# konstantineder/montecarlo-risk-engine

Measured on AMD Instinct MI355X. Metric: path-steps/sec at 1M paths x 250 steps; PV/CVA rel-error vs CPU ref, higher is better.
Workload: dtype f64

## Files before the change

montecarlo-risk-engine_amd/csrc/k1_paths.hip:

```cpp
#include "mcx_device.h"

namespace {


#ifndef MCX_K1_PPL
#define MCX_K1_PPL 1
#endif
template <int NSLOT, int NZ, bool INJECT, int SIG>
__global__ __launch_bounds__(MCX_BLOCK) void k1_paths(const K1Args a)
{
    constexpr int PPL = INJECT ? 1 : MCX_K1_PPL;
    __shared__ double bm_lds[INJECT ? 2 : MCX_BM_LDS_DOUBLES];
    const double* tab = nullptr;
    if (!INJECT) { mcx_bm_load(bm_lds); tab = bm_lds; }
    const int64_t tid = (int64_t)blockIdx.x * MCX_BLOCK + threadIdx.x;
    const int64_t half = (int64_t)gridDim.x * MCX_BLOCK;
    if (tid >= a.n) return;
    double reg[PPL][2 * NSLOT];
    int64_t idx[PPL];
    bool live[PPL];
#pragma unroll
    for (int q = 0; q < PPL; ++q) {
        idx[q] = tid + q * half;
        live[q] = idx[q] < a.n;
        if (!live[q]) idx[q] = a.n - 1;
        sim_init_state<NSLOT, SIG>(a, reg[q], idx[q]);
    }
    for (int t = 0; t < a.n_initial_store; ++t)
#pragma unroll
        for (int q = 0; q < PPL; ++q) if (live[q]) sim_store_state<NSLOT, SIG>(a, t, idx[q], reg[q]);
    const mcx_bm_coef bc = mcx_bm_coef_load();
    const mcx_bm_vconst vc = mcx_bm_vconst_make(bc);
    for (int k = 0; k < a.n_steps; ++k) {
        int st;
        if constexpr (INJECT || SIG == SIG_GENERIC) {
#pragma unroll
            for (int q = 0; q < PPL; ++q)
                sim_substep<NSLOT, NZ, INJECT, SIG>(a, k, a.path_offset + (uint64_t)idx[q], idx[q], reg[q], tab, a.seed, bc, &vc);
            st = ldk(&a.steps[k].store_idx);
        } else {
            const StepData<NSLOT, NZ> sdat = sim_step_load<NSLOT, NZ, SIG>(a, k);
            __builtin_amdgcn_sched_barrier(0);
            uint64_t path[PPL];
            uint32_t st_q[PPL];
            double zz[PPL][NZ], uu[PPL];
#pragma unroll
            for (int q = 0; q < PPL; ++q) { path[q] = a.path_offset + (uint64_t)idx[q]; st_q[q] = (uint32_t)k; }
            const bool rare = sim_draw_n<PPL, NZ, SIG, 7>(a, st_q, path, zz, uu, tab, a.seed, bc, vc);
            if (__builtin_expect(__any(rare), 0)) {
#pragma unroll
                for (int q = 0; q < PPL; ++q) sim_draw<NZ, false, SIG, 7, true>(a, k, path[q], idx[q], zz[q], uu[q], tab, a.seed, bc, &vc);
            }
            st = -1;
#pragma unroll
            for (int q = 0; q < PPL; ++q) st = sim_apply_loaded<NSLOT, NZ, SIG>(a, sdat, reg[q], zz[q], uu[q]);
        }
        if (st >= 0)
#pragma unroll
            for (int q = 0; q < PPL; ++q) if (live[q]) sim_store_state<NSLOT, SIG>(a, st, idx[q], reg[q], a.aux + (int64_t)k * NSLOT * MCX_AUX);
    }
}

template <int NSLOT, int NZ, int SIG>
int launch_k1(const K1Args& a, bool inject, hipStream_t s)
{
    const int ppl = inject ? 1 : MCX_K1_PPL;
    const int grid = (int)((a.n + (int64_t)MCX_BLOCK * ppl - 1) / ((int64_t)MCX_BLOCK * ppl));
    if (inject) hipLaunchKernelGGL((k1_paths<NSLOT, NZ, true, SIG>), dim3(grid), dim3(MCX_BLOCK), 0, s, a);
    else hipLaunchKernelGGL((k1_paths<NSLOT, NZ, false, SIG>), dim3(grid), dim3(MCX_BLOCK), 0, s, a);
    return 0;
}

__global__ __launch_bounds__(MCX_BLOCK) void k1_rng_draws(uint64_t seed, uint64_t path0, int64_t n, uint32_t step, uint32_t draw,
                                                          uint32_t* __restrict__ words, double* __restrict__ u, double* __restrict__ z)
{
    __shared__ double bm_lds[MCX_BM_LDS_DOUBLES];
    mcx_bm_load(bm_lds);
    const mcx_bm_coef bc = mcx_bm_coef_load();
    for (int64_t i = (int64_t)blockIdx.x * MCX_BLOCK + threadIdx.x; i < n; i += (int64_t)gridDim.x * MCX_BLOCK) {
        const uint64_t path = path0 + (uint64_t)i;
        if (words) {
            uint32_t w0, w1, w2, w3;
            philox4x32_10((uint32_t)path, (uint32_t)(path >> 32), step, draw, (uint32_t)seed, (uint32_t)(seed >> 32), w0, w1, w2, w3);
            words[i] = w0; words[n + i] = w1; words[2 * n + i] = w2; words[3 * n + i] = w3;
            if (u) { u[i] = u53(w0, w1); u[n + i] = u53(w2, w3); }
        }
        if (z) {
            double ua, z0, z1;
            draw_pair<true>(seed, path, step, draw, ua, z0, z1, bm_lds, bc);
            z[i] = z0; z[n + i] = z1;
        }
    }
}

template <int BMB>
__global__ __launch_bounds__(MCX_BLOCK) void k1_box_muller(const uint32_t* __restrict__ words, int64_t n, double* __restrict__ u,
                                                          double* __restrict__ z)
{
    __shared__ double bm_lds[MCX_BM_LDS_DOUBLES_B(BMB)];
    mcx_bm_load<BMB>(bm_lds);
    const mcx_bm_coef bc = mcx_bm_coef_load();
    const mcx_bm_vconst vc = mcx_bm_vconst_make<BMB>(bc);
    for (int64_t i = (int64_t)blockIdx.x * MCX_BLOCK + threadIdx.x; i < n; i += (int64_t)gridDim.x * MCX_BLOCK) {
        const uint32_t w0 = words[i], w1 = words[n + i], w2 = words[2 * n + i], w3 = words[3 * n + i];
        double ua, z0, z1;
        pair_from_words<true, BMB>(w0, w1, w2, w3, ua, z0, z1, bm_lds, bc, &vc);
        if (u) { u[i] = ua; u[n + i] = u53(w2, w3); }
        z[i] = z0; z[n + i] = z1;
    }
}

}

extern "C" int mcx_box_muller(mcx_handle* h, const uint32_t* d_words, int64_t n, int32_t table_bits, double* d_u, double* d_z, void* stream)
{
    if (!h || !d_words || !d_z) return -1;
    if (table_bits != 7 && table_bits != 10) MCX_FAIL(h, -2, "mcx_box_muller: table_bits must be 7 or 10");
    if (n <= 0) return 0;
    const int grid = mcx_grid_for(n, MCX_BLOCK, 2048);
    if (table_bits == 7) hipLaunchKernelGGL(k1_box_muller<7>, dim3(grid), dim3(MCX_BLOCK), 0, (hipStream_t)stream, d_words, n, d_u, d_z);
    else hipLaunchKernelGGL(k1_box_muller<10>, dim3(grid), dim3(MCX_BLOCK), 0, (hipStream_t)stream, d_words, n, d_u, d_z);
    MCX_HIP(h, hipGetLastError());
    return 0;
}

extern "C" int mcx_rng_draws(mcx_handle* h, uint64_t seed, uint64_t path0, int64_t n, uint32_t step, uint32_t draw,
                             uint32_t* d_words, double* d_u, double* d_z, void* stream)
{
    if (!h) return -1;
    if (n <= 0) return 0;
    if (d_u && !d_words) MCX_FAIL(h, -2, "mcx_rng_draws: d_u needs d_words");
// ... 149 lines not shown
```

montecarlo-risk-engine_amd/csrc/kf_lean.hip:

```cpp
#include <cstdlib>
#include <map>
#include <utility>

#include "kf_common.h"

namespace {

template <int NSLOT, int PPL>
__device__ __forceinline__ void lean_date_cva(const FastDateCvaLds* __restrict__ rp, const double (&reg)[PPL][2 * NSLOT], double (&cva)[PPL],
                                              const double* __restrict__ etab)
{
    const mcx_expq_coef ec = mcx_expq_load(mcx_region_zero());
    const FastDateCvaLds r = *rp;
    double xe[2 * PPL], ev[2 * PPL];
#pragma unroll
    for (int q = 0; q < PPL; ++q) {
        xe[2 * q] = fma(r.m_s1, reg[q][FDC_S_REG], fma(r.m_n1, reg[q][FDC_NI_REG], r.m_c0));
        xe[2 * q + 1] = fma(r.c_c1, reg[q][FDC_C_REG], r.c_c0);
    }
    mcx_exp_tab_n<2 * PPL>(xe, ev, etab, ec);
#pragma unroll
    for (int q = 0; q < PPL; ++q) {
        const double x = fma(r.x_d, reg[q][FDC_X_REG], r.x_a);
        double p = 0.0;
        p += fma(fma(r.row0[2], x, r.row0[1]), x, r.row0[0]);
        p += fma(fma(r.row1[2], x, r.row1[1]), x, r.row1[0]);
        const double w = r.m_b * ev[2 * q];
        const double cs = fma(r.c_b, ev[2 * q + 1], r.c_a);
        cva[q] = fma(fmax(p, 0.0), w * (1.0 - cs), cva[q]);
    }
}

#define MCX_LEAN_WAVES 4
template <int NSLOT, int NZ, bool INJECT, int SIG, int PPL, bool SIMULATE, int DK = 0>
__global__ __launch_bounds__(MCX_BLOCK, MCX_LEAN_WAVES) void kf_lean(const FusedArgs)
{
    static_assert(DK == 0 || (SIG == SIG_VAS_CIR_E && SIMULATE && !INJECT), "the cva-date kernel simulates the Vasicek + CIR++ signature");
    constexpr int NREG = 2 * NSLOT;
    constexpr int TILE = MCX_BLOCK * PPL;
    extern __shared__ double lds[];
    KArgs& a0 = kargs_region(0);
    const int n_rec = a0.n_rec;
    const int64_t n = a0.k1.n;
    for (int q = threadIdx.x; q < 9 * n_rec; q += MCX_BLOCK) lds[q] = 0.0;
    FastDateCvaLds* const dlds = (FastDateCvaLds*)(lds + ((9 * n_rec + 1) & ~1));
    if constexpr (DK == 1) {
        const FastDateCva* __restrict__ dc = a0.cva_dates;
        const double* __restrict__ cf = a0.coeffs;
        const int n_dates = a0.n_dates;
        for (int q = threadIdx.x; q < 16 * n_dates; q += MCX_BLOCK) {
            const int t = q >> 4, e = q & 15;
            double v;
            if (e < FDC_HEAD) {
                v = ((const double*)(dc + t))[e];
            } else {
                const int off = e < FDC_HEAD + 3 ? dc[t].coeff_off0 : dc[t].coeff_off1;
                v = off >= 0 ? cf[off + (e - FDC_HEAD) % 3] : 0.0;
            }
            ((double*)dlds)[q] = v;
        }
    }
    constexpr int BMB = SIG == SIG_VAS_CIR_E ? 10 : 7;
    constexpr int BM = (INJECT || !SIMULATE) ? 0 : MCX_BM_LDS_DOUBLES_B(BMB);
    __shared__ double tab_lds[BM + MCX_EXP_LDS_DOUBLES];
    const double* tab = nullptr;
    const double* etab = tab_lds + BM;
    mcx_exp_tab_load(tab_lds + BM);
    if (BM) { mcx_bm_load<BMB>(tab_lds); tab = tab_lds; }
    __syncthreads();
    const int64_t tiles = (n + TILE - 1) / TILE;
    double n_block = 0.0;

    for (int64_t tile = blockIdx.x; tile < tiles; tile += gridDim.x) {
        const bool first_tile = tile == (int64_t)blockIdx.x;
        int64_t i[PPL];
        bool live[PPL];
        uint64_t path[PPL];
        double reg[PPL][NREG];
        double cfs[PPL], cva[PPL];
        int est[PPL];
        int n_init, n_steps;
        {
            KArgs& a = kargs_region(mcx_region_zero());
            const auto& k = a.k1;
#pragma unroll
            for (int q = 0; q < PPL; ++q) {
                const int64_t i_raw = tile * TILE + q * MCX_BLOCK + threadIdx.x;
                live[q] = i_raw < n;
                i[q] = live[q] ? i_raw : n - 1;
                path[q] = k.path_offset + (uint64_t)i[q];
                sim_init_state<NSLOT, SIG>(k, reg[q]);
                cfs[q] = 0.0; cva[q] = 0.0;
                est[q] = a.init_state[0];
            }
            const int64_t rest = n - tile * TILE;
            n_block += (double)(rest < TILE ? rest : TILE);
            n_init = k.n_initial_store; n_steps = k.n_steps;
        }
        if (SIMULATE) {
        int step = 0, t_init = 0;
#pragma unroll 1
        while (true) {
            const bool init = t_init < n_init;
            if (!init && step >= n_steps) break;
            int st = init ? t_init : -1;
            t_init += init ? 1 : 0;
            {
                const int zr0 = mcx_region_zero();
                const auto& k = kargs_region(zr0).k1;
                const uint64_t seed = k.seed;
                const mcx_bm_coef bc = mcx_bm_coef_load(zr0);
                const mcx_bm_vconst vc = mcx_bm_vconst_make<BMB>(bc);
#pragma unroll 1
                while (st < 0 && step < n_steps) {
                    if constexpr (SIG == SIG_GENERIC) {
#pragma unroll
                        for (int q = 0; q < PPL; ++q) sim_substep<NSLOT, NZ, INJECT, SIG, BMB, true>(k, step, path[q], i[q], reg[q], tab, seed, bc, &vc);
                        st = ldk(&k.steps[step].store_idx);
                    } else {
                        double zz[PPL][NZ], uu[PPL];
                        bool rare = false;
                        const StepData<NSLOT, NZ> sdat = sim_step_load<NSLOT, NZ, SIG>(k, step);
                        __builtin_amdgcn_sched_barrier(0);
                        if constexpr (INJECT) {
#pragma unroll
                            for (int q = 0; q < PPL; ++q) sim_draw<NZ, true, SIG, BMB>(k, step, path[q], i[q], zz[q], uu[q], tab, seed, bc, &vc);
                        } else {
                            uint32_t st_q[PPL];
#pragma unroll
                            for (int q = 0; q < PPL; ++q) st_q[q] = (uint32_t)step;
                            rare = sim_draw_n<PPL, NZ, SIG, BMB>(k, st_q, path, zz, uu, tab, seed, bc, vc);
                        }
                        if (!INJECT && __builtin_expect(__any(rare), 0)) {
#pragma unroll
                            for (int q = 0; q < PPL; ++q) sim_draw<NZ, false, SIG, BMB, true>(k, step, path[q], i[q], zz[q], uu[q], tab, seed, bc, &vc);
                        }
#pragma unroll
                        for (int q = 0; q < PPL; ++q) st = sim_apply_loaded<NSLOT, NZ, SIG, true>(k, sdat, reg[q], zz[q], uu[q]);
                    }
                    ++step;
                }
            }
            if (st >= 0) {
                if constexpr (DK == 1) lean_date_cva<NSLOT, PPL>(dlds + st, reg, cva, etab);
                else lean_date<NSLOT, SIG, PPL, true>(st, i, live, first_tile, lds, reg, cfs, cva, est, etab);
            }
        }
        } else {
            auto load_row = [&](int t, double (&dst)[PPL][NREG]) {
                const auto& k = kargs_region(0).k1;
                const int D = k.n_state;
#pragma unroll
                for (int q = 0; q < PPL; ++q)
#pragma unroll
                    for (int sl = 0; sl < NSLOT; ++sl) {
                        const bool bs = sig_kind(SIG, sl) >= 0 ? sig_is_bs(SIG, sl) : (k.slots[sl].kind == MCX_MODEL_BS);
                        const int c = k.slots[sl].state_off;
                        dst[q][2 * sl] = k.paths[((int64_t)t * D + c) * k.ld + i[q]];
                        dst[q][2 * sl + 1] = bs ? 0.0 : k.paths[((int64_t)t * D + c + 1) * k.ld + i[q]];
                    }
            };
            const int n_dates = kargs_region(0).n_dates;
            double bufb[PPL][NREG];
            load_row(0, reg);
            load_row(n_dates > 1 ? 1 : 0, bufb);
#pragma unroll 1
            for (int t = 0; t < n_dates; t += 2) {
                lean_date<NSLOT, SIG, PPL, false>(t, i, live, first_tile, lds, reg, cfs, cva, est, etab);
                if (t + 2 < n_dates) load_row(t + 2, reg);
                if (t + 1 < n_dates) {
                    lean_date<NSLOT, SIG, PPL, false>(t + 1, i, live, first_tile, lds, bufb, cfs, cva, est, etab);
                    if (t + 3 < n_dates) load_row(t + 3, bufb);
                }
            }
        }
        {
            KArgs& a = kargs_region(mcx_region_zero());
#pragma unroll
            for (int q = 0; q < PPL; ++q) if (a.cfs && live[q]) a.cfs[i[q]] = cfs[q];
            if (a.rec_pv[0] >= 0) lean_record<PPL>(cfs, live, a.rec_pv[0], n_rec, first_tile, lds);
            if (a.rec_cva[0] >= 0) {
                const double lgd = a.lgd[0];
                double cc[PPL];
#pragma unroll
                for (int q = 0; q < PPL; ++q) cc[q] = cva[q] * lgd;
                lean_record<PPL>(cc, live, a.rec_cva[0], n_rec, first_tile, lds);
            }
        }
    }
    __syncthreads();
    for (int r = threadIdx.x; r < n_rec; r += MCX_BLOCK) {
        double s1 = 0.0, s2 = 0.0;
        for (int w = 0; w < 4; ++w) { s1 += lds[n_rec + (w * n_rec + r) * 2]; s2 += lds[n_rec + (w * n_rec + r) * 2 + 1]; }
        double* dst = a0.partials + ((int64_t)blockIdx.x * n_rec + r) * 4;
        dst[0] = n_block; dst[1] = lds[r]; dst[2] = s1; dst[3] = s2;
    }
}

template <int NSLOT, int NZ, int SIG, int PPL>
int launch_lean_shape(const FusedArgs& a, int n_cu, bool inject, bool simulate, hipStream_t s)
{
    const int64_t tiles = (a.k1.n + MCX_BLOCK * PPL - 1) / (MCX_BLOCK * PPL);
    const size_t lds = sizeof(double) * (size_t)((9 * a.n_rec + 1) & ~1);
    const size_t lds_cva = lds + sizeof(FastDateCvaLds) * (size_t)a.n_dates;
    auto residency = [&](auto kernel, size_t bytes) {
        thread_local std::map<std::pair<const void*, size_t>, int> cache;
        const auto key = std::make_pair((const void*)kernel, bytes);
        auto it = cache.find(key);
        if (it == cache.end()) {
            int per_cu = 0;
            if (hipOccupancyMaxActiveBlocksPerMultiprocessor(&per_cu, kernel, MCX_BLOCK, bytes) != hipSuccess || per_cu < 1) per_cu = 1;
            it = cache.emplace(key, per_cu < MCX_LEAN_WAVES ? per_cu : MCX_LEAN_WAVES).first;
        }
        return (int64_t)it->second * n_cu;
    };
    auto sized = [&](int64_t resident) {
        if (tiles <= resident) return (int)tiles;
        const int64_t per = (tiles + resident - 1) / resident;
        return (int)((tiles + per - 1) / per);
    };
    int grid;
    if (!simulate) {
        auto kern = kf_lean<NSLOT, NZ, false, SIG, PPL, false>;
        grid = sized(residency(kern, lds));
// ... 73 lines not shown
```

montecarlo-risk-engine_amd/csrc/mcx_device.h:

```cpp
#pragma once
#include "mcx_internal.h"

struct K1Args {
    mcx_slot slots[MCX_MAX_SLOTS];
    double init_state[MCX_MAX_STATE];
    const mcx_step* __restrict__ steps;
    const double* __restrict__ chol;
    const double* __restrict__ aux;
    double* __restrict__ paths;
    const double* __restrict__ inject_z;
    const double* __restrict__ inject_u;
    const double* __restrict__ init_paths;
    int64_t n, ld;
    uint64_t seed, path_offset;
    int32_t scheme, n_steps, n_state, n_initial_store, flags, n_uniform;
};

static inline void mcx_fill_k1_args(const mcx_sim* sim, uint64_t seed, uint64_t path_offset, int64_t n_paths, int64_t ld,
                                    double* d_paths, const double* d_inject_z, const double* d_inject_u, K1Args* a)
{
    const mcx_sim_desc& d = sim->desc;
    memset(a, 0, sizeof(*a));
    for (int s = 0; s < d.n_slots; ++s) a->slots[s] = d.slots[s];
    for (int c = 0; c < d.n_state; ++c) a->init_state[c] = d.init_state[c];
    a->steps = sim->d_steps; a->chol = sim->d_chol; a->aux = sim->d_aux;
    a->paths = d_paths; a->inject_z = d_inject_z; a->inject_u = d_inject_u;
    a->n = n_paths; a->ld = ld; a->seed = seed; a->path_offset = path_offset;
    a->scheme = d.scheme; a->n_steps = d.n_steps; a->n_state = d.n_state; a->n_initial_store = d.n_initial_store;
    a->flags = d.flags; a->n_uniform = d.n_uniform;
}

__device__ __forceinline__ void philox4x32_10(uint32_t c0, uint32_t c1, uint32_t c2, uint32_t c3, uint32_t k0, uint32_t k1,
                                              uint32_t& o0, uint32_t& o1, uint32_t& o2, uint32_t& o3)
{
#pragma unroll
    for (int r = 0; r < 10; ++r) {
        const uint64_t p0 = (uint64_t)0xD2511F53u * c0;
        const uint64_t p1 = (uint64_t)0xCD9E8D57u * c2;
        const uint32_t n0 = __builtin_amdgcn_bitop3_b32((uint32_t)(p1 >> 32), c1, k0, 0x96);
        const uint32_t n2 = __builtin_amdgcn_bitop3_b32((uint32_t)(p0 >> 32), c3, k1, 0x96);
        c1 = (uint32_t)p1;
        c3 = (uint32_t)p0;
        c0 = n0;
        c2 = n2;
        k0 += 0x9E3779B9u;
        k1 += 0xBB67AE85u;
    }
    o0 = c0; o1 = c1; o2 = c2; o3 = c3;
}

__device__ __forceinline__ double u53(uint32_t lo, uint32_t hi, const mcx_bm_vconst* vc = nullptr)
{
    if (vc) return fma((double)hi, vc->s32, fma((double)(lo >> 11), vc->s53, vc->c54));
    return fma((double)hi, 0x1.0p-32, fma((double)(lo >> 11), 0x1.0p-53, 0x1.0p-54));
}

struct DevBridge {
    uint64_t seed, path_offset;
    const double* const* inject;
    int64_t ld;
};

__device__ __forceinline__ double dev_barrier_event(const DevEvent& e, const DevTerm* __restrict__ terms, const double* __restrict__ coeffs,
                                                    const DevBridge* __restrict__ bridge, const double* __restrict__ paths, int64_t D,
                                                    int64_t ld, int64_t i, double num)
{
    const int types = (int)e.aux[3];
    const int t1 = types & 7, t2 = types >> 3;
    const bool with_bridge = e.aux[0] == 5.0;
    double mx = -1.0e300, mn = 1.0e300, keep1 = 1.0, keep2 = 1.0, prev1 = 0.0, prev2 = 0.0;
    double c = 0.0;
    int draw_id = 0;
    DevBridge br = {0, 0, nullptr, 0};
    const double* __restrict__ inj = nullptr;
    if (with_bridge) {
        c = ldk(coeffs + e.coeff_off);
        draw_id = (int)ldk(coeffs + e.coeff_off + 1);
        br = ldk_struct(bridge);
        if (br.inject) inj = br.inject[draw_id];
    }
    AtomCache bc = {-1, -1, 0.0};
    for (int j = e.term_begin; j < e.term_end; ++j) {
        const double s = dev_atom_cached(ldk_struct(&terms[j]).atom, paths, D, ld, i, bc);
        mx = fmax(mx, s); mn = fmin(mn, s);
        if (with_bridge) {
            const double cur1 = mcx_log(s / e.aux[1]), cur2 = t2 ? mcx_log(s / e.aux[2]) : 0.0;
            if (j > e.term_begin) {
                const int k = j - e.term_begin - 1;
                for (int bi = 0; bi < (t2 ? 2 : 1); ++bi) {
                    const double p = mcx_exp(c * (bi ? prev2 * cur2 : prev1 * cur1));
                    double u;
                    if (inj) u = inj[(int64_t)(2 * k + bi) * br.ld + i];
                    else {
                        uint32_t w0, w1, w2, w3;
                        const uint64_t path = br.path_offset + (uint64_t)i;
                        philox4x32_10((uint32_t)path, (uint32_t)(path >> 32), (uint32_t)k, 0x80000000u | (uint32_t)(2 * draw_id + bi),
                                      (uint32_t)br.seed, (uint32_t)(br.seed >> 32), w0, w1, w2, w3);
                        u = u53(w0, w1);
                    }
                    const double hit = fmin(fmax((p - u + 0.05) / 0.1, 0.0), 1.0);
                    if (bi) keep2 *= 1.0 - hit; else keep1 *= 1.0 - hit;
                }
            }
            prev1 = cur1; prev2 = cur2;
        }
    }
    double pay = fmax(e.sign * (dev_atom(e.x, paths, D, ld, i) - e.strike), 0.0) * dev_barrier_ind(t1, e.aux[1], mx, mn);
    if (with_bridge) pay *= (t1 <= 2) ? keep1 : 1.0 - keep1;
    if (t2) {
        pay *= dev_barrier_ind(t2, e.aux[2], mx, mn);
        if (with_bridge) pay *= (t2 <= 2) ? keep2 : 1.0 - keep2;
    }
    return pay / num;
}

template <bool TAB = false, int BMB = 7, bool GUARD = true>
__device__ __forceinline__ bool pair_from_words(uint32_t w0, uint32_t w1, uint32_t w2, uint32_t w3, double& ua, double& z0, double& z1,
                                                const double* __restrict__ tab, const mcx_bm_coef& bc, const mcx_bm_vconst* vc = nullptr)
{
    ua = u53(w0, w1, vc);
    double s, c, r;
    if (TAB) {
        const double r2 = mcx_m2log_tab<BMB>(ua, tab, bc, vc);
        if (!GUARD) r = mcx_sqrt_gp(r2);
        else if (__builtin_expect(__any(w1 == 0xffffffffu), 0)) r = ua < 1.0 ? mcx_sqrt_g(r2) : 0.0;
        else r = mcx_sqrt_gp(r2);
        const int j = (int)(w3 >> (32 - BMB));
        const double ur = u53(w2, w3 & ((1u << (32 - BMB)) - 1u), vc);
        mcx_sincos2pi_tab<BMB>(ur, j, tab, s, c, bc, vc);
    } else {
        r = mcx_sqrt(-2.0 * mcx_log(ua));
        mcx_sincos2pi(u53(w2, w3), s, c);
    }
    z0 = r * c;
    z1 = r * s;
    return w1 == 0xffffffffu;
}

template <bool TAB = false, int BMB = 7, bool GUARD = true>
__device__ __forceinline__ bool draw_pair(uint64_t seed, uint64_t path, uint32_t step, uint32_t draw, double& ua, double& z0, double& z1,
                                          const double* __restrict__ tab, const mcx_bm_coef& bc, const mcx_bm_vconst* vc = nullptr)
{
    uint32_t w0, w1, w2, w3;
    philox4x32_10((uint32_t)path, (uint32_t)(path >> 32), step, draw, (uint32_t)seed, (uint32_t)(seed >> 32), w0, w1, w2, w3);
    return pair_from_words<TAB, BMB, GUARD>(w0, w1, w2, w3, ua, z0, z1, tab, bc, vc);
}

template <bool TAB = false>
__device__ __forceinline__ void draw_pair(uint64_t seed, uint64_t path, uint32_t step, uint32_t draw, double& ua, double& z0, double& z1,
                                          const double* __restrict__ tab = nullptr)
{
    const mcx_bm_coef bc = mcx_bm_coef_load();
    draw_pair<TAB>(seed, path, step, draw, ua, z0, z1, tab, bc);
}

__device__ __forceinline__ double degree_of_truth(double x, bool fuzzy, double eps)
{
    if (!fuzzy) return x > 0.0 ? 1.0 : 0.0;
    const double v = (x + eps) / (2.0 * eps);
    return fmin(fmax(v, 0.0), 1.0);
}

struct AuxPtr {
    const double* __restrict__ p;
    __device__ __forceinline__ double operator[](int i) const { return ldk(p + i); }
    __device__ __forceinline__ mcx_aux_drv drv() const { return ldk_struct((const mcx_aux_drv*)(p + MCX_AUX_C0)); }
};
struct AuxRegs {
    double v[MCX_AUX];
    __device__ __forceinline__ double operator[](int i) const { return v[i]; }
    __device__ __forceinline__ mcx_aux_drv drv() const { mcx_aux_drv d; d.c0 = v[MCX_AUX_C0]; d.c1 = v[MCX_AUX_C1]; d.c2 = v[MCX_AUX_C2]; return d; }
};

template <int KIND, int SCHEME, bool POS = false, class SL, class AUX>
__device__ __forceinline__ void step_slot(const SL& sl, int scheme_rt, int flags, double dt, double sq,
                                          const AUX& aux, double& s0, double& s1, double zc0, double zc1, double u)
{
    const auto* p = sl.p;
    const int scheme = SCHEME >= 0 ? SCHEME : scheme_rt;
    switch (KIND >= 0 ? KIND : sl.kind) {
    case MCX_MODEL_BS:
        if (scheme == MCX_SCHEME_ANALYTICAL) {
            s0 = s0 * mcx_exp(aux[0] + (zc0 - aux[1]));
        } else {
            const mcx_aux_drv dc = aux.drv();
            s0 = fma(s0, fma(dc.c2, zc0, dc.c0), s0);
        }
        break;
    case MCX_MODEL_VASICEK: {
        const double r = s0;
        s1 = s1 + r * dt;
        if (scheme == MCX_SCHEME_ANALYTICAL) s0 = (p[2] + (r - p[2]) * aux[0]) + zc0;
        else {
            const mcx_aux_drv dc = aux.drv();
            s0 = fma(dc.c1, r, s0);
            s0 = fma(dc.c2, zc0, s0);
            s0 = s0 + dc.c0;
        }
        break;
    }
    case MCX_MODEL_HW: {
        const double r = s0;
        s1 = s1 + r * dt;
        if (scheme == MCX_SCHEME_ANALYTICAL) s0 = r * aux[0] + aux[1] + zc0;
        else s0 = r + (aux[0] - p[3] * r) * dt + p[1] * sq * zc0;
        break;
    }
    case MCX_MODEL_CIRPP: {
        const double y = s0;
        const double sy = POS ? mcx_sqrt_gp(y) : mcx_sqrt_g(y);
        const mcx_aux_drv dc = aux.drv();
// ... 68 lines not shown
    default: break;
    }
}


enum { SIG_GENERIC = 0, SIG_VAS_CIR_E = 1, SIG_BS_A = 2, SIG_BS_E = 3, SIG_HESTON_QE = 4, SIG_HESTON_E = 5,
       SIG_VAS_E = 6, SIG_VAS_A = 7, SIG_BS_VAS_CIRDET_E = 8 };

__host__ __device__ constexpr int sig_kind(int sig, int slot)
{
    return sig == SIG_VAS_CIR_E ? (slot == 0 ? MCX_MODEL_VASICEK : MCX_MODEL_CIRPP)
         : (sig == SIG_BS_A || sig == SIG_BS_E) ? MCX_MODEL_BS
         : (sig == SIG_HESTON_QE || sig == SIG_HESTON_E) ? MCX_MODEL_HESTON
         : (sig == SIG_VAS_E || sig == SIG_VAS_A) ? MCX_MODEL_VASICEK
         : sig == SIG_BS_VAS_CIRDET_E ? (slot == 0 ? MCX_MODEL_BS : slot == 1 ? MCX_MODEL_VASICEK : MCX_MODEL_CIRPP_DET)
         : -1;
}
__host__ __device__ constexpr int sig_scheme(int sig)
{
    return (sig == SIG_VAS_CIR_E || sig == SIG_BS_E || sig == SIG_HESTON_E || sig == SIG_VAS_E || sig == SIG_BS_VAS_CIRDET_E) ? MCX_SCHEME_EULER
         : (sig == SIG_BS_A || sig == SIG_VAS_A) ? MCX_SCHEME_ANALYTICAL
         : sig == SIG_HESTON_QE ? MCX_SCHEME_QE : -1;
}
__host__ __device__ constexpr bool sig_is_bs(int sig, int slot) { return sig_kind(sig, slot) == MCX_MODEL_BS; }

static inline int mcx_sim_signature(const mcx_sim_desc& d)
{
    auto k = [&](int s) { return d.slots[s].kind; };
    if (d.n_slots == 2 && k(0) == MCX_MODEL_VASICEK && k(1) == MCX_MODEL_CIRPP && d.scheme == MCX_SCHEME_EULER) return SIG_VAS_CIR_E;
    if (d.n_slots == 3 && k(0) == MCX_MODEL_BS && k(1) == MCX_MODEL_VASICEK && k(2) == MCX_MODEL_CIRPP_DET && d.scheme == MCX_SCHEME_EULER)
        return SIG_BS_VAS_CIRDET_E;
    if (d.n_slots == 1) {
        if (k(0) == MCX_MODEL_BS) return d.scheme == MCX_SCHEME_ANALYTICAL ? SIG_BS_A : d.scheme == MCX_SCHEME_EULER ? SIG_BS_E : SIG_GENERIC;
        if (k(0) == MCX_MODEL_HESTON) return d.scheme == MCX_SCHEME_QE ? SIG_HESTON_QE : d.scheme == MCX_SCHEME_EULER ? SIG_HESTON_E : SIG_GENERIC;
        if (k(0) == MCX_MODEL_VASICEK) return d.scheme == MCX_SCHEME_EULER ? SIG_VAS_E : d.scheme == MCX_SCHEME_ANALYTICAL ? SIG_VAS_A : SIG_GENERIC;
    }
    return SIG_GENERIC;
}

__device__ __forceinline__ AuxPtr aux_of_slot(const double* __restrict__ ax, int s) { return AuxPtr{ax + s * MCX_AUX}; }
template <int NSLOT>
__device__ __forceinline__ const AuxRegs& aux_of_slot(const AuxRegs (&ax)[NSLOT], int s) { return ax[s]; }

template <int NSLOT, int NZ, int SIG, int S, bool POS = false, class KA, class AX>
__device__ __forceinline__ void step_slots(const KA& k, const mcx_step& sp, const AX& ax,
                                           double (&reg)[2 * NSLOT], const double (&zc)[NZ], double u)
{
    if constexpr (S < NSLOT) {
        const double zc0 = (NSLOT == 1) ? zc[0] : zc[S < NZ ? S : 0];
        const double zc1 = (NSLOT == 1 && NZ > 1) ? zc[NZ > 1 ? 1 : 0] : 0.0;
        step_slot<sig_kind(SIG, S), sig_scheme(SIG), POS>(k.slots[S], k.scheme, k.flags | k.slots[S].flags, sp.dt, sp.sqrt_dt,
                                                      aux_of_slot(ax, S), reg[2 * S], reg[2 * S + 1], zc0, zc1, u);
        step_slots<NSLOT, NZ, SIG, S + 1, POS>(k, sp, ax, reg, zc, u);
    }
}

template <int NZ, bool INJECT, int SIG, int BMB = 7, bool GUARD = true, class KA>
__device__ __forceinline__ bool sim_draw(const KA& k, int step, uint64_t path, int64_t i, double (&z)[NZ], double& u,
                                         const double* __restrict__ tab, uint64_t seed, const mcx_bm_coef& bc, const mcx_bm_vconst* vc = nullptr)
{
    u = 0.0;
    bool rare = false;
    if (INJECT) {
#pragma unroll
        for (int j = 0; j < NZ; ++j) z[j] = k.inject_z[((int64_t)step * NZ + j) * k.ld + i];
        if (k.n_uniform) u = k.inject_u[(int64_t)step * k.ld + i];
    } else {
        double ua;
#pragma unroll
        for (int q = 0; q < (NZ + 1) / 2; ++q) {
            double z0, z1;
            rare |= draw_pair<true, BMB, GUARD>(seed, path, (uint32_t)step, (uint32_t)q, ua, z0, z1, tab, bc, vc);
            z[2 * q] = z0;
            if (2 * q + 1 < NZ) z[2 * q + 1] = z1;
        }
        if (sig_scheme(SIG) == MCX_SCHEME_QE || (sig_scheme(SIG) < 0 && k.n_uniform)) {
            double z0, z1;
            draw_pair<false>(seed, path, (uint32_t)step, (uint32_t)((NZ + 1) / 2), u, z0, z1, nullptr, bc);
        }
    }
    return rare;
}

template <int PPL>
__device__ __forceinline__ void philox4x32_10_n(const uint64_t (&path)[PPL], const uint32_t (&step)[PPL], uint32_t draw, uint64_t seed,
                                                uint32_t (&o0)[PPL], uint32_t (&o1)[PPL], uint32_t (&o2)[PPL], uint32_t (&o3)[PPL])
{
    uint32_t c0[PPL], c1[PPL], c2[PPL], c3[PPL];
#pragma unroll
    for (int q = 0; q < PPL; ++q) { c0[q] = (uint32_t)path[q]; c1[q] = (uint32_t)(path[q] >> 32); c2[q] = step[q]; c3[q] = draw; }
    uint32_t k0 = (uint32_t)seed, k1 = (uint32_t)(seed >> 32);
#pragma unroll
    for (int r = 0; r < 10; ++r) {
#pragma unroll
        for (int q = 0; q < PPL; ++q) {
            const uint64_t p0 = (uint64_t)0xD2511F53u * c0[q];
            const uint64_t p1 = (uint64_t)0xCD9E8D57u * c2[q];
            const uint32_t n0 = __builtin_amdgcn_bitop3_b32((uint32_t)(p1 >> 32), c1[q], k0, 0x96);
            const uint32_t n2 = __builtin_amdgcn_bitop3_b32((uint32_t)(p0 >> 32), c3[q], k1, 0x96);
            c1[q] = (uint32_t)p1; c3[q] = (uint32_t)p0; c0[q] = n0; c2[q] = n2;
        }
        k0 += 0x9E3779B9u;
        k1 += 0xBB67AE85u;
    }
#pragma unroll
    for (int q = 0; q < PPL; ++q) { o0[q] = c0[q]; o1[q] = c1[q]; o2[q] = c2[q]; o3[q] = c3[q]; }
}

template <int PPL, int BMB>
__device__ __forceinline__ bool draw_pairs_staged(uint64_t seed, const uint64_t (&path)[PPL], const uint32_t (&step)[PPL], uint32_t draw,
                                                  double (&z0)[PPL], double (&z1)[PPL], const double* __restrict__ tab,
                                                  const mcx_bm_coef& C, const mcx_bm_vconst& vc)
{
    constexpr int N = 1 << BMB, LOG_TERMS = mcx_bm_shape<BMB>::LOG_TERMS;
    uint32_t w0[PPL], w1[PPL], w2[PPL], w3[PPL];
    philox4x32_10_n<PPL>(path, step, draw, seed, w0, w1, w2, w3);
    double m[PPL], ed[PPL], ps[PPL], pc[PPL];
    int e[PPL];
    mcx_d2 tc[PPL], sc[PPL];
#pragma unroll
    for (int q = 0; q < PPL; ++q) {
        const double ua = u53(w0[q], w1[q], &vc);
        m[q] = __builtin_amdgcn_frexp_mant(ua);
        e[q] = __builtin_amdgcn_frexp_exp(ua);
        const int jl = (__double2hiint(m[q]) >> (20 - BMB)) & (N - 1);
        tc[q] = ((const mcx_d2*)tab)[jl];
        sc[q] = ((const mcx_d2*)(tab + 2 * N))[(int)(w3[q] >> (32 - BMB))];
    }
    __builtin_amdgcn_sched_barrier(0);
#pragma unroll
    for (int q = 0; q < PPL; ++q) {
        const double ur = u53(w2[q], w3[q] & ((1u << (32 - BMB)) - 1u), &vc);
        const double d = fma(ur, 6.28318530717958647692, vc.trig_off);
        const double d2 = d * d;
        double qs, qc;
        if constexpr (mcx_bm_shape<BMB>::TRIG_TERMS == 3) {
            qs = fma(fma(vc.sin_head, d2, C.c[7]), d2, C.c[6]);
            qc = fma(fma(vc.cos_head, d2, C.c[10]), d2, C.c[9]);
        } else {
            qs = fma(vc.sin_head, d2, C.c[6]);
            qc = fma(vc.cos_head, d2, C.c[9]);
        }
        ps[q] = fma(d * d2, qs, d);
        pc[q] = fma(d2, qc, 1.0);
        ed[q] = (double)e[q];
    }
    __builtin_amdgcn_sched_barrier(0);
    bool rare = false;
#pragma unroll
    for (int q = 0; q < PPL; ++q) {
        const double s = fma(m[q], tc[q].x, 2.0);
        double p = vc.log_head;
#pragma unroll
        for (int k = LOG_TERMS - 2; k >= 0; --k) p = fma(p, s, C.c[k]);
        const double r2 = fma(ed[q], -2.0 * 6.93147180559945309417e-01, tc[q].y) + fma(s * s, p, s);
        const double r = mcx_sqrt_gp(r2);
        const double sn = fma(sc[q].x, pc[q], sc[q].y * ps[q]);
        const double cs = fma(-sc[q].x, ps[q], sc[q].y * pc[q]);
        z0[q] = r * cs;
        z1[q] = r * sn;
        rare |= w1[q] == 0xffffffffu;
    }
    return rare;
}

template <int PPL, int NZ, int SIG, int BMB, class KA>
__device__ __forceinline__ bool sim_draw_n(const KA& k, const uint32_t (&step)[PPL], const uint64_t (&path)[PPL], double (&z)[PPL][NZ], double (&u)[PPL],
                                           const double* __restrict__ tab, uint64_t seed, const mcx_bm_coef& bc, const mcx_bm_vconst& vc)
{
    bool rare = false;
#pragma unroll
    for (int dq = 0; dq < (NZ + 1) / 2; ++dq) {
        double a[PPL], b[PPL];
        rare |= draw_pairs_staged<PPL, BMB>(seed, path, step, (uint32_t)dq, a, b, tab, bc, vc);
#pragma unroll
        for (int q = 0; q < PPL; ++q) { z[q][2 * dq] = a[q]; if (2 * dq + 1 < NZ) z[q][2 * dq + 1] = b[q]; }
    }
#pragma unroll
    for (int q = 0; q < PPL; ++q) {
        u[q] = 0.0;
        if (sig_scheme(SIG) == MCX_SCHEME_QE || (sig_scheme(SIG) < 0 && k.n_uniform)) {
            double t0, t1;
            draw_pair<false>(seed, path[q], step[q], (uint32_t)((NZ + 1) / 2), u[q], t0, t1, nullptr, bc);
        }
    }
    return rare;
}

template <int NSLOT, int NZ, int SIG, bool POS = false, class KA>
__device__ __forceinline__ int sim_apply(const KA& k, int step, double (&reg)[2 * NSLOT], const double (&z)[NZ], double u)
{
    const mcx_step sp = ldk_struct(&k.steps[step]);
    double zc[NZ];
    constexpr bool UNIT_L00 = sig_scheme(SIG) == MCX_SCHEME_EULER || sig_scheme(SIG) == MCX_SCHEME_QE;
    const double* __restrict__ L = UNIT_L00 ? k.chol : k.chol + (int64_t)sp.chol_idx * NZ * NZ;
#pragma unroll
    for (int r = 0; r < NZ; ++r) {
        double acc = (UNIT_L00 && r == 0) ? z[0] : ldk(L + r * NZ) * z[0];
#pragma unroll
        for (int c = 1; c <= r; ++c) acc = fma(ldk(L + r * NZ + c), z[c], acc);
        zc[r] = acc;
    }
    const double* __restrict__ ax = k.aux + (int64_t)step * NSLOT * MCX_AUX;
    step_slots<NSLOT, NZ, SIG, 0, POS>(k, sp, ax, reg, zc, u);
    return sp.store_idx;
}

template <int NSLOT, int NZ>
struct StepData {
    mcx_step sp;
    double L[NZ * NZ];
    AuxRegs ax[NSLOT];
};
template <int NSLOT, int NZ, int SIG, class KA>
__device__ __forceinline__ StepData<NSLOT, NZ> sim_step_load(const KA& k, int step)
{
    StepData<NSLOT, NZ> d;
    d.sp = ldk_struct(&k.steps[step]);
    constexpr bool UNIT_L00 = sig_scheme(SIG) == MCX_SCHEME_EULER || sig_scheme(SIG) == MCX_SCHEME_QE;
    const double* __restrict__ L = UNIT_L00 ? k.chol : k.chol + (int64_t)d.sp.chol_idx * NZ * NZ;
#pragma unroll
    for (int q = 0; q < NZ * NZ; ++q) d.L[q] = ldk(L + q);
    struct P2 { double v[2]; };
    struct P4 { double v[4]; };
    static_assert(MCX_AUX == 8, "aux row layout");
    const double* __restrict__ ax = k.aux + (int64_t)step * NSLOT * MCX_AUX;
#pragma unroll
    for (int s = 0; s < NSLOT; ++s) {
        const P2 a = ldk_struct((const P2*)(ax + s * MCX_AUX)), b = ldk_struct((const P2*)(ax + s * MCX_AUX + 2));
        const P4 c = ldk_struct((const P4*)(ax + s * MCX_AUX + 4));
        d.ax[s].v[0] = a.v[0]; d.ax[s].v[1] = a.v[1]; d.ax[s].v[2] = b.v[0]; d.ax[s].v[3] = b.v[1];
#pragma unroll
        for (int q = 0; q < 4; ++q) d.ax[s].v[4 + q] = c.v[q];
    }
    return d;
}
template <int NSLOT, int NZ, int SIG, bool POS = false, class KA>
__device__ __forceinline__ int sim_apply_loaded(const KA& k, const StepData<NSLOT, NZ>& d, double (&reg)[2 * NSLOT], const double (&z)[NZ], double u)
{
    double zc[NZ];
    constexpr bool UNIT_L00 = sig_scheme(SIG) == MCX_SCHEME_EULER || sig_scheme(SIG) == MCX_SCHEME_QE;
#pragma unroll
    for (int r = 0; r < NZ; ++r) {
        double acc = (UNIT_L00 && r == 0) ? z[0] : d.L[r * NZ] * z[0];
#pragma unroll
        for (int c = 1; c <= r; ++c) acc = fma(d.L[r * NZ + c], z[c], acc);
        zc[r] = acc;
    }
    step_slots<NSLOT, NZ, SIG, 0, POS>(k, d.sp, d.ax, reg, zc, u);
    return d.sp.store_idx;
}

template <int NSLOT, int NZ, bool INJECT, int SIG, int BMB = 7, bool POS = false, class KA>
__device__ __forceinline__ void sim_substep(const KA& k, int step, uint64_t path, int64_t i, double (&reg)[2 * NSLOT],
                                            const double* __restrict__ tab, uint64_t seed, const mcx_bm_coef& bc, const mcx_bm_vconst* vc = nullptr)
{
    double z[NZ], u;
// ... 47 lines not shown
```

montecarlo-risk-engine_amd/csrc/mcx_math.h:

```cpp
#pragma once

__device__ const double MCX_EXP_C[14] __attribute__((aligned(64))) = {1.00000000000000000e+00, 1.00000000000000000e+00, 5.00000000000000000e-01, 1.66666666666666657e-01, 4.16666666666666644e-02, 8.33333333333333322e-03, 1.38888888888888894e-03, 1.98412698412698413e-04, 2.48015873015873016e-05, 2.75573192239858925e-06, 2.75573192239858883e-07, 2.50521083854417202e-08, 2.08767569878681002e-09, 1.60590438368216133e-10};
__device__ const double MCX_SIN_C[10] = {3.14159265358979312e+00, -5.16771278004997026e+00, 2.55016403987734552e+00, -5.99264529320792105e-01, 8.21458866111282326e-02, -7.37043094571435044e-03, 4.66302805767612554e-04, -2.19153534478302173e-05, 7.95205400147551261e-07, -2.29484289972698730e-08};
__device__ const double MCX_COS_C[10] = {1.00000000000000000e+00, -4.93480220054467900e+00, 4.05871212641676848e+00, -1.33526276885458950e+00, 2.35330630358893206e-01, -2.58068913900140612e-02, 1.92957430940392314e-03, -1.04638104924845705e-04, 4.30306958703294729e-06, -1.38789524622137714e-07};
__device__ const double MCX_LOG_C[7] = {6.666666666666735130e-01, 3.999999999940941908e-01, 2.857142874366239149e-01, 2.222219843214978396e-01, 1.818357216161805012e-01, 1.531383769920937332e-01, 1.479819860511658591e-01};

__device__ __forceinline__ int mcx_region_zero()
{
    int z;
    asm volatile("s_mov_b32 %0, 0" : "=s"(z));
    return z;
}
__device__ __forceinline__ uint32_t mcx_region_copy(uint32_t v)
{
    uint32_t o;
    asm volatile("s_mov_b32 %0, %1" : "=s"(o) : "s"(v));
    return o;
}

struct mcx_exp_coef { double c[14]; };
__device__ __forceinline__ mcx_exp_coef mcx_exp_load(int z = 0)
{
    return ldk_struct((const mcx_exp_coef*)(MCX_EXP_C + z));
}
// ... 54 lines not shown
    ps *= r;
    const int q = (int)n;
    const bool swap = q & 1;
    const double a = swap ? pc : ps, b = swap ? ps : pc;
    s = (q & 2) ? -a : a;
    c = ((q + 1) & 2) ? -b : b;
}

__device__ __forceinline__ double mcx_rcp(double d)
{
    double r = __builtin_amdgcn_rcp(d);
    r = fma(fma(-d, r, 1.0), r, r);
    r = fma(fma(-d, r, 1.0), r, r);
    return r;
}

__device__ __forceinline__ double mcx_sqrt(double a)
{
    const double y = __builtin_amdgcn_rsq(a);
    double g = a * y, h = 0.5 * y;
    const double r = fma(-h, g, 0.5);
    g = fma(g, r, g);
    h = fma(h, r, h);
    const double d = fma(-g, g, a);
    g = fma(d, h, g);
    return a > 0.0 ? g : 0.0;
}

__device__ __forceinline__ double mcx_sqrt_h(double a, double& h_out)
{
    const double y = __builtin_amdgcn_rsq(a);
    double g = a * y, h = 0.5 * y;
    const double r = fma(-h, g, 0.5);
    g = fma(g, r, g);
    h = fma(h, r, h);
    const double d = fma(-g, g, a);
    g = fma(d, h, g);
    h_out = a <= 0.0 ? __builtin_huge_val() : h;
    return a <= 0.0 ? 0.0 : g;
}

__device__ __forceinline__ double mcx_sqrt_g(double a)
{
    const double y = __builtin_amdgcn_rsq(a);
    double g = a * y;
    const double h = 0.5 * y;
    const double r = fma(-h, g, 0.5);
    g = fma(g, r, g);
    return a <= 0.0 ? 0.0 : g;
}

__device__ __forceinline__ double mcx_sqrt_gp(double a)
{
    const double y = __builtin_amdgcn_rsq(a);
    const double g = a * y;
    const double h = 0.5 * y;
    return fma(g, fma(-h, g, 0.5), g);
}

#include "mcx_tables.h"
#define MCX_BM_LDS_DOUBLES_B(BMB) (4 << (BMB))
#define MCX_BM_LDS_DOUBLES MCX_BM_LDS_DOUBLES_B(7)
template <int BMB> struct mcx_bm_shape;
template <> struct mcx_bm_shape<7> {
    static constexpr int LOG_TERMS = 6, TRIG_TERMS = 3;
    static __device__ __forceinline__ double log_src(int q) { return MCX_LOG_TAB[q]; }
    static __device__ __forceinline__ double trig_src(int q) { return MCX_TRIG_TAB[q]; }
};
template <> struct mcx_bm_shape<10> {
    static constexpr int LOG_TERMS = 4, TRIG_TERMS = 2;
    static __device__ __forceinline__ double log_src(int q) { return MCX_LOG_TAB_L[q]; }
    static __device__ __forceinline__ double trig_src(int q) { return MCX_TRIG_TAB_L[q]; }
};

__device__ const double MCX_BM_C[12] __attribute__((aligned(64))) = {0.25, (1.0 / 3.0) * 0.25, 0.03125, 0.2 * 0.0625, (1.0 / 6.0) * 0.03125, (1.0 / 7.0) * 0.015625,
                                                                     -1.0 / 6.0, 1.0 / 120.0, -1.0 / 5040.0, -0.5, 1.0 / 24.0, -1.0 / 720.0};
struct mcx_bm_coef { double c[12]; };
__device__ __forceinline__ mcx_bm_coef mcx_bm_coef_load(int z = 0)
{
    return ldk_struct((const mcx_bm_coef*)(MCX_BM_C + z));
}

struct mcx_bm_vconst {
    double c54;
    double s53, s32;
    double log_head;
    double sin_head, cos_head;
    double trig_off;
};
__device__ __forceinline__ double mcx_opaque_v(double x) { asm volatile("" : "+v"(x)); return x; }
__device__ __forceinline__ double mcx_opaque_s(double x) { asm volatile("" : "+s"(x)); return x; }
template <int BMB = 7>
__device__ __forceinline__ mcx_bm_vconst mcx_bm_vconst_make(const mcx_bm_coef& C)
{
    using SH = mcx_bm_shape<BMB>;
    mcx_bm_vconst v;
    v.c54 = mcx_opaque_v(0x1.0p-54); v.s53 = mcx_opaque_s(0x1.0p-53); v.s32 = mcx_opaque_s(0x1.0p-32);
    v.log_head = mcx_opaque_v(C.c[SH::LOG_TERMS - 1]);
    v.sin_head = mcx_opaque_v(C.c[5 + SH::TRIG_TERMS]);
    v.cos_head = mcx_opaque_v(C.c[8 + SH::TRIG_TERMS]);
    v.trig_off = mcx_opaque_v(-3.14159265358979323846 / (double)(1 << BMB));
    return v;
}

template <int BMB = 7>
__device__ __forceinline__ void mcx_bm_load(double* __restrict__ tab)
{
    constexpr int N = 1 << BMB;
    for (int q = threadIdx.x; q < 2 * N; q += blockDim.x) {
        tab[q] = -2.0 * mcx_bm_shape<BMB>::log_src(q);
        tab[2 * N + q] = mcx_bm_shape<BMB>::trig_src(q);
    }
    __syncthreads();
}

typedef double mcx_d2 __attribute__((ext_vector_type(2)));

template <int BMB = 7>
__device__ __forceinline__ double mcx_m2log_tab(double x, const double* __restrict__ tab, const mcx_bm_coef& C, const mcx_bm_vconst* vc = nullptr)
{
    constexpr int N = 1 << BMB, LOG_TERMS = mcx_bm_shape<BMB>::LOG_TERMS;
    const double m = __builtin_amdgcn_frexp_mant(x);
    const int e = __builtin_amdgcn_frexp_exp(x);
    const int j = (__double2hiint(m) >> (20 - BMB)) & (N - 1);
    const mcx_d2 tc = ((const mcx_d2*)tab)[j];
    const double s = fma(m, tc.x, 2.0);
    double q = vc ? vc->log_head : C.c[LOG_TERMS - 1];
#pragma unroll
    for (int k = LOG_TERMS - 2; k >= 0; --k) q = fma(q, s, C.c[k]);
    const double p = fma(s * s, q, s);
    return fma((double)e, -2.0 * 6.93147180559945309417e-01, tc.y) + p;
}

template <int BMB = 7>
__device__ __forceinline__ void mcx_sincos2pi_tab(double ur, int j, const double* __restrict__ tab, double& s, double& c, const mcx_bm_coef& C,
                                                  const mcx_bm_vconst* vc = nullptr)
{
    constexpr int N = 1 << BMB;
    const double d = fma(ur, 6.28318530717958647692, vc ? vc->trig_off : -3.14159265358979323846 / (double)N);
    const mcx_d2 sc = ((const mcx_d2*)(tab + 2 * N))[j];
    const double d2 = d * d;
    double qs, qc;
    if constexpr (mcx_bm_shape<BMB>::TRIG_TERMS == 3) {
        qs = fma(fma(vc ? vc->sin_head : C.c[8], d2, C.c[7]), d2, C.c[6]);
        qc = fma(fma(vc ? vc->cos_head : C.c[11], d2, C.c[10]), d2, C.c[9]);
    } else {
        qs = fma(vc ? vc->sin_head : C.c[7], d2, C.c[6]);
        qc = fma(vc ? vc->cos_head : C.c[10], d2, C.c[9]);
    }
    const double ps = fma(d * d2, qs, d);
    const double pc = fma(d2, qc, 1.0);
    s = fma(sc.x, pc, sc.y * ps);
    c = fma(-sc.x, ps, sc.y * pc);
}

#define MCX_EXP_LDS_DOUBLES 128
__device__ const double MCX_EXPQ_C[4] __attribute__((aligned(32))) = {0.5, 1.0 / 6.0, 1.0 / 24.0, 1.0 / 120.0};
struct mcx_expq_coef { double c[4]; };
__device__ __forceinline__ mcx_expq_coef mcx_expq_load(int z = 0) { return ldk_struct((const mcx_expq_coef*)(MCX_EXPQ_C + z)); }

__device__ __forceinline__ void mcx_exp_tab_load(double* __restrict__ tab)
{
    for (int q = threadIdx.x; q < MCX_EXP_LDS_DOUBLES; q += blockDim.x) tab[q] = MCX_EXP2_TAB[q];
}

__device__ __forceinline__ double mcx_exp_tab(double x, const double* __restrict__ tab, const mcx_expq_coef& C)
{
    const double k = rint(x * MCX_128_LN2);
    double r = fma(k, -MCX_LN2_128_HI, x);
    r = fma(k, -MCX_LN2_128_LO, r);
    const int ki = (int)k;
    const double T = tab[ki & 127];
    double q = fma(C.c[3], r, C.c[2]);
    q = fma(q, r, C.c[1]);
    q = fma(q, r, C.c[0]);
    q = fma(q, r, 1.0);
    q *= r;
    return ldexp(fma(T, q, T), ki >> 7);
}

// ... 27 lines not shown
```

Measured before the change: 290.5 billion.

## Specialize Philox first rounds for uniform path-high word and use bit-trick uniforms

```diff
diff --git a/montecarlo-risk-engine_amd/csrc/k1_paths.hip b/montecarlo-risk-engine_amd/csrc/k1_paths.hip
--- a/montecarlo-risk-engine_amd/csrc/k1_paths.hip
+++ b/montecarlo-risk-engine_amd/csrc/k1_paths.hip
@@ -46,7 +46,7 @@
             double zz[PPL][NZ], uu[PPL];
 #pragma unroll
             for (int q = 0; q < PPL; ++q) { path[q] = a.path_offset + (uint64_t)idx[q]; st_q[q] = (uint32_t)k; }
-            const bool rare = sim_draw_n<PPL, NZ, SIG, 7>(a, st_q, path, zz, uu, tab, a.seed, bc, vc);
+            const bool rare = sim_draw_n<PPL, NZ, SIG, 7>(a, st_q, path, 0u, zz, uu, tab, a.seed, bc, vc);
             if (__builtin_expect(__any(rare), 0)) {
 #pragma unroll
                 for (int q = 0; q < PPL; ++q) sim_draw<NZ, false, SIG, 7, true>(a, k, path[q], idx[q], zz[q], uu[q], tab, a.seed, bc, &vc);
diff --git a/montecarlo-risk-engine_amd/csrc/kf_lean.hip b/montecarlo-risk-engine_amd/csrc/kf_lean.hip
--- a/montecarlo-risk-engine_amd/csrc/kf_lean.hip
+++ b/montecarlo-risk-engine_amd/csrc/kf_lean.hip
@@ -1,5 +1,6 @@
 #include <cstdlib>
 #include <map>
+#include <type_traits>
 #include <utility>
 
 #include "kf_common.h"
@@ -38,6 +39,7 @@
     static_assert(DK == 0 || (SIG == SIG_VAS_CIR_E && SIMULATE && !INJECT), "the cva-date kernel simulates the Vasicek + CIR++ signature");
     constexpr int NREG = 2 * NSLOT;
     constexpr int TILE = MCX_BLOCK * PPL;
+    constexpr bool STAGED = SIG != SIG_GENERIC && !INJECT;
     extern __shared__ double lds[];
     KArgs& a0 = kargs_region(0);
     const int n_rec = a0.n_rec;
@@ -111,6 +113,11 @@
                 const uint64_t seed = k.seed;
                 const mcx_bm_coef bc = mcx_bm_coef_load(zr0);
                 const mcx_bm_vconst vc = mcx_bm_vconst_make<BMB>(bc);
+                const uint64_t base = k.path_offset + (uint64_t)(tile * TILE);
+                const uint32_t path_hi = (uint32_t)(base >> 32);
+                const bool hi_uniform = path_hi == (uint32_t)((base + (TILE - 1)) >> 32);
+                auto run = [&](auto hu) {
+                constexpr bool HU = decltype(hu)::value;
 #pragma unroll 1
                 while (st < 0 && step < n_steps) {
                     if constexpr (SIG == SIG_GENERIC) {
@@ -129,7 +136,7 @@
                             uint32_t st_q[PPL];
 #pragma unroll
                             for (int q = 0; q < PPL; ++q) st_q[q] = (uint32_t)step;
-                            rare = sim_draw_n<PPL, NZ, SIG, BMB>(k, st_q, path, zz, uu, tab, seed, bc, vc);
+                            rare = sim_draw_n<PPL, NZ, SIG, BMB, HU>(k, st_q, path, path_hi, zz, uu, tab, seed, bc, vc);
                         }
                         if (!INJECT && __builtin_expect(__any(rare), 0)) {
 #pragma unroll
@@ -140,6 +147,9 @@
                     }
                     ++step;
                 }
+                };
+                if (STAGED && hi_uniform) run(std::true_type{});
+                else run(std::false_type{});
             }
             if (st >= 0) {
                 if constexpr (DK == 1) lean_date_cva<NSLOT, PPL>(dlds + st, reg, cva, etab);
diff --git a/montecarlo-risk-engine_amd/csrc/mcx_device.h b/montecarlo-risk-engine_amd/csrc/mcx_device.h
--- a/montecarlo-risk-engine_amd/csrc/mcx_device.h
+++ b/montecarlo-risk-engine_amd/csrc/mcx_device.h
@@ -49,10 +49,29 @@
     o0 = c0; o1 = c1; o2 = c2; o3 = c3;
 }
 
+__device__ __forceinline__ double two52_plus(uint32_t m_hi, uint32_t m_lo)
+{
+    return __hiloint2double((int)(0x43300000u | m_hi), (int)m_lo);
+}
+
+__device__ __forceinline__ double u53_exact(double two52_m, const mcx_bm_vconst* vc)
+{
+    return vc ? fma(two52_m, vc->s53, vc->cu) : fma(two52_m, 0x1.0p-53, -0x1.fffffffffffffp-2);
+}
+
 __device__ __forceinline__ double u53(uint32_t lo, uint32_t hi, const mcx_bm_vconst* vc = nullptr)
 {
-    if (vc) return fma((double)hi, vc->s32, fma((double)(lo >> 11), vc->s53, vc->c54));
-    return fma((double)hi, 0x1.0p-32, fma((double)(lo >> 11), 0x1.0p-53, 0x1.0p-54));
+    const double inner = u53_exact(two52_plus(0u, lo >> 11), vc);
+    return fma((double)hi, vc ? vc->s32 : 0x1.0p-32, inner);
+}
+
+template <int BMB>
+__device__ __forceinline__ double u53_rem(uint32_t lo, uint32_t hi, const mcx_bm_vconst* vc = nullptr)
+{
+    static_assert(BMB >= 1 && BMB <= 21, "u53_rem: 1 <= BMB <= 21");
+    asm("" : "+v"(hi));
+    const uint32_t m_hi = __builtin_amdgcn_ubfe(hi, 11, 21 - BMB);
+    return u53_exact(two52_plus(m_hi, __builtin_amdgcn_alignbit(hi, lo, 11)), vc);
 }
 
 struct DevBridge {
@@ -126,7 +145,7 @@
         else if (__builtin_expect(__any(w1 == 0xffffffffu), 0)) r = ua < 1.0 ? mcx_sqrt_g(r2) : 0.0;
         else r = mcx_sqrt_gp(r2);
         const int j = (int)(w3 >> (32 - BMB));
-        const double ur = u53(w2, w3 & ((1u << (32 - BMB)) - 1u), vc);
+        const double ur = u53_rem<BMB>(w2, w3, vc);
         mcx_sincos2pi_tab<BMB>(ur, j, tab, s, c, bc, vc);
     } else {
         r = mcx_sqrt(-2.0 * mcx_log(ua));
@@ -361,16 +380,11 @@
     return rare;
 }
 
-template <int PPL>
-__device__ __forceinline__ void philox4x32_10_n(const uint64_t (&path)[PPL], const uint32_t (&step)[PPL], uint32_t draw, uint64_t seed,
-                                                uint32_t (&o0)[PPL], uint32_t (&o1)[PPL], uint32_t (&o2)[PPL], uint32_t (&o3)[PPL])
-{
-    uint32_t c0[PPL], c1[PPL], c2[PPL], c3[PPL];
-#pragma unroll
-    for (int q = 0; q < PPL; ++q) { c0[q] = (uint32_t)path[q]; c1[q] = (uint32_t)(path[q] >> 32); c2[q] = step[q]; c3[q] = draw; }
-    uint32_t k0 = (uint32_t)seed, k1 = (uint32_t)(seed >> 32);
-#pragma unroll
-    for (int r = 0; r < 10; ++r) {
+template <int PPL, int R0>
+__device__ __forceinline__ void philox_rounds_n(uint32_t (&c0)[PPL], uint32_t (&c1)[PPL], uint32_t (&c2)[PPL], uint32_t (&c3)[PPL], uint32_t k0, uint32_t k1)
+{
+#pragma unroll
+    for (int r = R0; r < 10; ++r) {
 #pragma unroll
         for (int q = 0; q < PPL; ++q) {
             const uint64_t p0 = (uint64_t)0xD2511F53u * c0[q];
@@ -382,18 +396,50 @@
         k0 += 0x9E3779B9u;
         k1 += 0xBB67AE85u;
     }
-#pragma unroll
-    for (int q = 0; q < PPL; ++q) { o0[q] = c0[q]; o1[q] = c1[q]; o2[q] = c2[q]; o3[q] = c3[q]; }
-}
-
-template <int PPL, int BMB>
-__device__ __forceinline__ bool draw_pairs_staged(uint64_t seed, const uint64_t (&path)[PPL], const uint32_t (&step)[PPL], uint32_t draw,
-                                                  double (&z0)[PPL], double (&z1)[PPL], const double* __restrict__ tab,
+}
+
+template <int PPL>
+__device__ __forceinline__ void philox4x32_10_n(const uint64_t (&path)[PPL], const uint32_t (&step)[PPL], uint32_t draw, uint64_t seed,
+                                                uint32_t (&o0)[PPL], uint32_t (&o1)[PPL], uint32_t (&o2)[PPL], uint32_t (&o3)[PPL])
+{
+#pragma unroll
+    for (int q = 0; q < PPL; ++q) { o0[q] = (uint32_t)path[q]; o1[q] = (uint32_t)(path[q] >> 32); o2[q] = step[q]; o3[q] = draw; }
+    philox_rounds_n<PPL, 0>(o0, o1, o2, o3, (uint32_t)seed, (uint32_t)(seed >> 32));
+}
+
+template <int PPL>
+__device__ __forceinline__ void philox4x32_10_n(const uint64_t (&path)[PPL], uint32_t path_hi, const uint32_t (&step)[PPL], uint32_t draw,
+                                                uint64_t seed, uint32_t (&o0)[PPL], uint32_t (&o1)[PPL], uint32_t (&o2)[PPL], uint32_t (&o3)[PPL])
+{
+    const uint32_t k0 = (uint32_t)seed, k1 = (uint32_t)(seed >> 32);
+    const uint32_t k0b = k0 + 0x9E3779B9u, k1b = k1 + 0xBB67AE85u;
+#pragma unroll
+    for (int q = 0; q < PPL; ++q) {
+        const uint64_t p0 = (uint64_t)0xD2511F53u * (uint32_t)path[q];
+        const uint64_t p1 = (uint64_t)0xCD9E8D57u * step[q];
+        const uint32_t a0 = (uint32_t)(p1 >> 32) ^ path_hi ^ k0;
+        const uint32_t a1 = (uint32_t)p1;
+        const uint32_t a2 = (uint32_t)(p0 >> 32) ^ (draw ^ k1);
+        const uint32_t a3 = (uint32_t)p0;
+        const uint64_t r0 = (uint64_t)0xD2511F53u * a0;
+        const uint64_t r1 = (uint64_t)0xCD9E8D57u * a2;
+        o0[q] = (uint32_t)(r1 >> 32) ^ (a1 ^ k0b);
+        o2[q] = a3 ^ ((uint32_t)(r0 >> 32) ^ k1b);
+        o1[q] = (uint32_t)r1;
+        o3[q] = (uint32_t)r0;
+    }
+    philox_rounds_n<PPL, 2>(o0, o1, o2, o3, k0 + 2u * 0x9E3779B9u, k1 + 2u * 0xBB67AE85u);
+}
+
+template <int PPL, int BMB, bool HU = false>
+__device__ __forceinline__ bool draw_pairs_staged(uint64_t seed, const uint64_t (&path)[PPL], uint32_t path_hi, const uint32_t (&step)[PPL],
+                                                  uint32_t draw, double (&z0)[PPL], double (&z1)[PPL], const double* __restrict__ tab,
                                                   const mcx_bm_coef& C, const mcx_bm_vconst& vc)
 {
     constexpr int N = 1 << BMB, LOG_TERMS = mcx_bm_shape<BMB>::LOG_TERMS;
     uint32_t w0[PPL], w1[PPL], w2[PPL], w3[PPL];
-    philox4x32_10_n<PPL>(path, step, draw, seed, w0, w1, w2, w3);
+    if constexpr (HU) philox4x32_10_n<PPL>(path, path_hi, step, draw, seed, w0, w1, w2, w3);
+    else philox4x32_10_n<PPL>(path, step, draw, seed, w0, w1, w2, w3);
     double m[PPL], ed[PPL], ps[PPL], pc[PPL];
     int e[PPL];
     mcx_d2 tc[PPL], sc[PPL];
@@ -402,14 +448,14 @@
         const double ua = u53(w0[q], w1[q], &vc);
         m[q] = __builtin_amdgcn_frexp_mant(ua);
         e[q] = __builtin_amdgcn_frexp_exp(ua);
-        const int jl = (__double2hiint(m[q]) >> (20 - BMB)) & (N - 1);
-        tc[q] = ((const mcx_d2*)tab)[jl];
+        const uint32_t ol = ((uint32_t)__double2hiint(m[q]) >> (16 - BMB)) & (uint32_t)(16 * (N - 1));
+        tc[q] = *(const mcx_d2*)((const char*)tab + ol);
         sc[q] = ((const mcx_d2*)(tab + 2 * N))[(int)(w3[q] >> (32 - BMB))];
     }
     __builtin_amdgcn_sched_barrier(0);
 #pragma unroll
     for (int q = 0; q < PPL; ++q) {
-        const double ur = u53(w2[q], w3[q] & ((1u << (32 - BMB)) - 1u), &vc);
+        const double ur = u53_rem<BMB>(w2[q], w3[q], &vc);
         const double d = fma(ur, 6.28318530717958647692, vc.trig_off);
         const double d2 = d * d;
         double qs, qc;
@@ -443,15 +489,16 @@
     return rare;
 }
 
-template <int PPL, int NZ, int SIG, int BMB, class KA>
-__device__ __forceinline__ bool sim_draw_n(const KA& k, const uint32_t (&step)[PPL], const uint64_t (&path)[PPL], double (&z)[PPL][NZ], double (&u)[PPL],
-                                           const double* __restrict__ tab, uint64_t seed, const mcx_bm_coef& bc, const mcx_bm_vconst& vc)
+template <int PPL, int NZ, int SIG, int BMB, bool HU = false, class KA>
+__device__ __forceinline__ bool sim_draw_n(const KA& k, const uint32_t (&step)[PPL], const uint64_t (&path)[PPL], uint32_t path_hi, double (&z)[PPL][NZ],
+                                           double (&u)[PPL], const double* __restrict__ tab, uint64_t seed, const mcx_bm_coef& bc,
+                                           const mcx_bm_vconst& vc)
 {
     bool rare = false;
 #pragma unroll
     for (int dq = 0; dq < (NZ + 1) / 2; ++dq) {
         double a[PPL], b[PPL];
-        rare |= draw_pairs_staged<PPL, BMB>(seed, path, step, (uint32_t)dq, a, b, tab, bc, vc);
+        rare |= draw_pairs_staged<PPL, BMB, HU>(seed, path, path_hi, step, (uint32_t)dq, a, b, tab, bc, vc);
 #pragma unroll
         for (int q = 0; q < PPL; ++q) { z[q][2 * dq] = a[q]; if (2 * dq + 1 < NZ) z[q][2 * dq + 1] = b[q]; }
     }
diff --git a/montecarlo-risk-engine_amd/csrc/mcx_math.h b/montecarlo-risk-engine_amd/csrc/mcx_math.h
--- a/montecarlo-risk-engine_amd/csrc/mcx_math.h
+++ b/montecarlo-risk-engine_amd/csrc/mcx_math.h
@@ -160,7 +160,7 @@
 }
 
 struct mcx_bm_vconst {
-    double c54;
+    double cu;
     double s53, s32;
     double log_head;
     double sin_head, cos_head;
@@ -173,7 +173,7 @@
 {
     using SH = mcx_bm_shape<BMB>;
     mcx_bm_vconst v;
-    v.c54 = mcx_opaque_v(0x1.0p-54); v.s53 = mcx_opaque_s(0x1.0p-53); v.s32 = mcx_opaque_s(0x1.0p-32);
+    v.cu = mcx_opaque_v(-0x1.fffffffffffffp-2); v.s53 = mcx_opaque_s(0x1.0p-53); v.s32 = mcx_opaque_s(0x1.0p-32);
     v.log_head = mcx_opaque_v(C.c[SH::LOG_TERMS - 1]);
     v.sin_head = mcx_opaque_v(C.c[5 + SH::TRIG_TERMS]);
     v.cos_head = mcx_opaque_v(C.c[8 + SH::TRIG_TERMS]);
```

Result: faster. 297.2 billion (median of 6 runs) (+2.3%).
